# ByeongKyuPark/Depth-Aware-Shader-Effects-for-NeRF

Hardware: AMD Instinct MI355X
Metric: rays/sec at 800x800, 64 coarse + 128 fine samples (higher is better)
Workload: dtype fp32 (f16x3 split)

## Files before the change

depth-aware-shader-effects-for-nerf_amd/csrc/common.h:

```cpp
#pragma once
#include <hip/hip_runtime.h>
#include <stdint.h>
#include <stdio.h>
#include <utility>
#include "../../include/nerfmi_train.h"
#include "layout.h"

namespace nerf {

int set_error(int code, const char* fmt, ...);

inline int check_launch(const char* what) {
  hipError_t e = hipGetLastError();
  if (e != hipSuccess) return set_error(NERF_ERR_HIP, "%s: %s", what, hipGetErrorString(e));
  return NERF_OK;
}

typedef float f32x16 __attribute__((ext_vector_type(16)));
typedef float f32x4 __attribute__((ext_vector_type(4)));

template <typename F, int... Is>
__device__ __forceinline__ void static_for_impl(F&& f, std::integer_sequence<int, Is...>) {
  (f(std::integral_constant<int, Is>{}), ...);
}
template <int N, typename F>
__device__ __forceinline__ void static_for(F&& f) {
  static_for_impl(f, std::make_integer_sequence<int, N>{});
}

__host__ __device__ __forceinline__ int64_t imin64(int64_t a, int64_t b) { return a < b ? a : b; }

__device__ __forceinline__ float opaque_neg_one() {
  float v = -1.0f;
  asm("" : "+s"(v));
  return v;
}
__device__ __forceinline__ _Float16 split_lo(float x, _Float16 hi) {
  return (_Float16)__builtin_fmaf((float)hi, opaque_neg_one(), x);
}

__device__ __forceinline__ uint32_t split_lo_pair(uint32_t hi2, float x0, float x1) {
  uint32_t lo;
  asm("v_fma_mixlo_f16 %0, %1, -1.0, %2 op_sel_hi:[1,0,0]\n\t"
      "v_fma_mixhi_f16 %0, %1, -1.0, %3 op_sel:[1,0,0] op_sel_hi:[1,0,0]"
      : "=&v"(lo)
      : "v"(hi2), "v"(x0), "v"(x1));
  return lo;
}

constexpr int kRowStoreAux = 2;
constexpr int kRowLoadAux = 0;

typedef uint32_t u32x4s __attribute__((ext_vector_type(4)));
template <int AUX, bool PAD = false, typename V>
__device__ __forceinline__ void store16_rows(V v, __amdgpu_buffer_rsrc_t rows, uint32_t voff) {
  static_assert(sizeof(V) == 16, "16-byte stores");
  __builtin_amdgcn_raw_buffer_store_b128(__builtin_bit_cast(u32x4s, v), rows, (int)voff, 0, AUX);
  if constexpr (PAD) asm volatile("s_nop 1");
}

__device__ __forceinline__ float expf_rn(float x) { return (float)exp((double)x); }

__device__ __forceinline__ float wave_max_nn(float v) {
  v = fmaxf(v, __int_as_float(__builtin_amdgcn_mov_dpp(__float_as_int(v), 0xB1, 0xF, 0xF, false)));
  v = fmaxf(v, __int_as_float(__builtin_amdgcn_mov_dpp(__float_as_int(v), 0x4E, 0xF, 0xF, false)));
  v = fmaxf(v, __int_as_float(__builtin_amdgcn_mov_dpp(__float_as_int(v), 0x141, 0xF, 0xF, false)));
  v = fmaxf(v, __int_as_float(__builtin_amdgcn_mov_dpp(__float_as_int(v), 0x140, 0xF, 0xF, false)));
  const float r0 = __int_as_float(__builtin_amdgcn_readlane(__float_as_int(v), 0));
  const float r1 = __int_as_float(__builtin_amdgcn_readlane(__float_as_int(v), 16));
  const float r2 = __int_as_float(__builtin_amdgcn_readlane(__float_as_int(v), 32));
  const float r3 = __int_as_float(__builtin_amdgcn_readlane(__float_as_int(v), 48));
  return fmaxf(fmaxf(r0, r1), fmaxf(r2, r3));
}

__device__ __forceinline__ float block_exp_record(float m) {
  int e;
  frexpf(m, &e);
  return -(float)(kBlockExpBias + (m > 0.0f ? e : kBlockExpZero));
}

__device__ __forceinline__ float hash_uniform(uint64_t seed, uint64_t idx) {
  uint64_t z = seed + 0x9E3779B97F4A7C15ull * (idx + 1);
  z = (z ^ (z >> 30)) * 0xBF58476D1CE4E5B9ull;
  z = (z ^ (z >> 27)) * 0x94D049BB133111EBull;
  z ^= z >> 31;
  return (float)(z >> 40) * (1.0f / 16777216.0f);
}

__host__ __device__ __forceinline__ uint64_t rng_key_at(uint64_t seed, uint64_t first) {
  return seed + 0x9E3779B97F4A7C15ull * first;
}

int launch_get_rays(int H, int W, float focal, const float* c2w, int row0, int nrows,
                    float* o, float* d, hipStream_t s);
int launch_rng_uniforms(uint64_t seed, int64_t first, int64_t n, float* out, hipStream_t s);
int launch_pe(const float* x, int64_t M, int dims, int levels, int include_input, float* out, hipStream_t s);
int launch_normalize(const float* d, int64_t B, float* out, hipStream_t s);
int launch_stratified(const float* o, const float* d, int64_t B, float near_f, float span_f,
                      int N, const float* t_vals, int perturb, const float* t_rand,
                      uint64_t seed, float* z, float* pts, hipStream_t s);
int launch_importance(const float* o, const float* d, const float* z, const float* w,
                      int64_t B, int N, int Nf, const float* u_lin, const float* u_rand,
                      uint64_t seed, float* z_all, float* pts_all, const float* rgb_c, const float* sigma_c,
                      float* rgb_all, float* sigma_all, float* z_fine, int* fine_slot, hipStream_t s,
                      uint16_t* merged_src = nullptr);
int launch_pack(const float* const* params, float* packed, hipStream_t s);
int launch_ray_features(const float* packed, const float* dirs, int64_t R, const float* app,
                        int64_t app_rows, float* feat, hipStream_t s, float* encd = nullptr, float* dn_out = nullptr);
extern int g_mlp_arith;
int launch_mlp16(const float* packed, const float* o, const float* d, const float* z, int64_t R, int N,
                 const float* feat, float* rgb, float* sigma, const int* out_slot, int out_T, hipStream_t s,
                 float* save = nullptr, const float* encd = nullptr, uint32_t* masks = nullptr);
int launch_mlp16_live(const float* packed, const float* o, const float* d, const float* z, int N, const float* feat,
                      const float* encd, const int* live, int64_t M_live, float* rgb, float* sigma, float* rgb_live,
                      float* sigma_live, float* save, uint32_t* masks, hipStream_t s);
int launch_mlp16s(const float* packed, const float* o, const float* d, const float* z, int64_t R, int N,
                  const float* feat, float* rgb, float* sigma, const int* out_slot, int out_T, hipStream_t s);
int launch_mlp16s_live(const float* packed, const float* o, const float* d, const float* z, int64_t R, int N,
                       const float* feat, float* rgb, float* sigma, const int* live, const int* live_count,
                       hipStream_t s);
size_t occ_block_count_bytes(int64_t M);
int launch_occ_classify(const float* o, const float* d, const float* z, int64_t B, int n, const uint32_t* bits, int G,
                        const float* lo, const float* inv, int* live, int* live_count, uint8_t* mask,
                        float* sigma_zero, float* rgb_zero, uint32_t* block_counts, hipStream_t s);
int launch_occ_gather_grads(const float* dsigma, const float* drgb, const int* live, int64_t M_live,
                            float* dsigma_live, float* drgb_live, hipStream_t s);
int launch_occ_pack(const float* lattice, int G, int sp, float thr, uint32_t* bits, hipStream_t s);
int launch_occ_dilate(const uint32_t* in, int G, uint32_t* out, hipStream_t s);
int launch_mlp(const float* packed, const float* o, const float* d, const float* z, int64_t R,
               int N, const float* feat, float* rgb, float* sigma, const int* out_slot, int out_T,
               hipStream_t s, float* save = nullptr, const float* encd = nullptr, uint32_t* masks = nullptr);
struct CompositeSamples {
  const float *rgb, *sigma, *rgb_f, *sigma_f;
  const uint16_t* src;
  const float* z;
  int64_t B;
  int N, Nf;
  bool merged;
};
inline CompositeSamples dense_samples(const float* rgb, const float* sigma, const float* z, int64_t B, int N) {
  return {rgb, sigma, nullptr, nullptr, nullptr, z, B, N, 0, false};
}
inline CompositeSamples merged_samples(const float* rgb_c, const float* sigma_c, const float* rgb_f,
                                       const float* sigma_f, const uint16_t* src, const float* z_all, int64_t B, int N,
                                       int Nf) {
  return {rgb_c, sigma_c, rgb_f, sigma_f, src, z_all, B, N, Nf, true};
}
struct CompositeBg {
  const float* bg;
  int stride;
  float bd;
  float* acc_map;
};
int launch_composite(const CompositeSamples& in, float* rgb_map, float* depth, float* weights, const CompositeBg* bga,
                     hipStream_t s);

}
```

depth-aware-shader-effects-for-nerf_amd/csrc/mlp16s.hip:

```cpp
#include <atomic>
#include "common.h"
#include "pe_sin.h"
#include "stream16.h"

namespace nerf {

#ifdef NERF_MLP16S_STAMPS
__device__ unsigned long long nerf16s_stamps[65536][16];
constexpr int kSStampFloats = kW16Waves * 32;
constexpr int kSStampIter = 8;
#define STAMP16S_ASM(i, insn)                                                               \
  do {                                                                                      \
    __builtin_amdgcn_sched_barrier(0);                                                      \
    unsigned long long t_;                                                                  \
    asm volatile(insn " %0\n\ts_waitcnt lgkmcnt(0)" : "=s"(t_)::"memory");                 \
    __builtin_amdgcn_sched_barrier(0);                                                      \
    if (lane == 0 && stamp_on) reinterpret_cast<unsigned long long*>(lds + kSLdsFloats)[wave * 16 + (i)] = t_; \
  } while (0)
#define STAMP16S(i) STAMP16S_ASM(i, "s_memtime")
#define STAMP16S_REAL(i) STAMP16S_ASM(i, "s_memrealtime")
#else
constexpr int kSStampFloats = 0;
#define STAMP16S(i) do {} while (0)
#define STAMP16S_REAL(i) do {} while (0)
#endif

__device__ __forceinline__ f32x4 mfma16s(h16x8 a, h16x8 b, f32x4 c) {
  return __builtin_amdgcn_mfma_f32_16x16x32_f16(a, b, c, 0, 0, 0);
}

constexpr int kSLdsPe = 4 * kChunkFloats;
constexpr int kSLdsBias = kSLdsPe + kW16Waves * kPeSteps * 64;
constexpr int kSLdsSigmaW = kSLdsBias + 8 * kHidden;
constexpr int kSLdsVecFloats = 8 * kHidden + kHidden + 4;
constexpr int kSLdsConsts = kSLdsBias + kSLdsVecFloats;
constexpr int kSLdsRgb = kSLdsConsts + kS16Consts;
constexpr int kSLdsRgbFloats = 3 * kDirHidden + 4;
constexpr int kSLdsFeat = kSLdsRgb + kSLdsRgbFloats;
constexpr int kSLdsFloats = kSLdsFeat + kW16Waves * kRayFeat;
static_assert(kSLdsRgb % 4 == 0 && kSLdsFeat % 4 == 0, "LDS vector layout");
static_assert((kS16Chunks & (kS16Chunks - 1)) == 0 && kS16Chunks % 4 == 0, "the stream wraps onto the same ring slots");

typedef h16x8 STile[2][2];
typedef f32x4 SAcc[8][2][2];

template <int TI>
__device__ __forceinline__ void sread_tile(const float* slot, const uint32_t (&off)[2], STile& a) {
#pragma unroll
  for (int r = 0; r < 2; ++r)
#pragma unroll
    for (int part = 0; part < 2; ++part)
      a[r][part] = __builtin_bit_cast(h16x8, *reinterpret_cast<const f32x4*>(slot + off[r] + TI * 512 + part * 256));
}

template <int TI, int K>
__device__ __forceinline__ void sread_frag(const float* slot, const uint32_t (&off)[2], STile& a) {
  constexpr int r = K >> 1, part = K & 1;
  a[r][part] = __builtin_bit_cast(h16x8, *reinterpret_cast<const f32x4*>(slot + off[r] + TI * 512 + part * 256));
}

#ifdef NERF16S_PIECE_DMA
constexpr uint32_t kSDmaWave = 1024;
template <int SLOT, int I>
__device__ __forceinline__ void sdma_piece(const float* __restrict__ stream, int c, uint32_t lds_base, uint32_t voff) {
  chunk_dma_piece<SLOT, I>(stream, c, lds_base, voff);
}
#else
constexpr uint32_t kSDmaWave = 4096;
template <int SLOT, int I>
__device__ __forceinline__ void sdma_piece(const float* __restrict__ stream, int c, uint32_t lds_base, uint32_t voff) {
  const char* src = reinterpret_cast<const char*>(stream) + (size_t)c * (kChunkFloats * 4);
  if constexpr (I == 0)
    asm volatile(
        "s_mov_b32 m0, %2\n\t"
        "s_nop 0\n\t"
        "global_load_lds_dwordx4 %0, %1"
        :
        : "v"(voff), "s"(src), "s"(lds_base + SLOT * (kChunkFloats * 4))
        : "memory", "m0");
  else
    asm volatile("global_load_lds_dwordx4 %0, %1 offset:%2" : : "v"(voff), "s"(src), "n"(I * 1024) : "memory");
}
#endif
template <int SLOT>
__device__ __forceinline__ void sdma_chunk(const float* __restrict__ stream, int c, uint32_t lds_base, uint32_t voff) {
  sdma_piece<SLOT, 0>(stream, c, lds_base, voff);
  sdma_piece<SLOT, 1>(stream, c, lds_base, voff);
  sdma_piece<SLOT, 2>(stream, c, lds_base, voff);
  sdma_piece<SLOT, 3>(stream, c, lds_base, voff);
}

template <int G, int TI, bool FIRST, typename Hook>
__device__ __forceinline__ void smfma_tile(const STile& a, const Operand& b0, const Operand& b1, SAcc& acc,
                                           Hook&& hook) {
  static_for<4>([&](auto jc) __attribute__((always_inline)) {
    constexpr int j = decltype(jc)::value, r = j >> 1, st = j & 1;
    const Operand& b = st ? b1 : b0;
    f32x4 c;
    if constexpr (FIRST) c = mfma16s(a[r][1], b.hi, f32x4{});
    else c = mfma16s(a[r][1], b.hi, acc[4 * G + TI][r][st]);
    c = mfma16s(a[r][0], b.lo, c);
    acc[4 * G + TI][r][st] = mfma16s(a[r][0], b.hi, c);
    hook(jc);
  });
}

constexpr int kSValuGap0 = 5;
template <int G, int TI, bool FIRST, int NRD, int VPG, typename Reads, typename Side, typename Hook>
__device__ __forceinline__ void ssegment(const STile& a, const Operand& b0, const Operand& b1, SAcc& acc, Reads&& reads,
                                         Side&& side, Hook&& hook) {
  side(std::integral_constant<int, 0>{});
  __builtin_amdgcn_sched_barrier(0);
  reads();
  smfma_tile<G, TI, FIRST>(a, b0, b1, acc, hook);
  side(std::integral_constant<int, 1>{});
#pragma unroll
  for (int i = 0; i < 12; ++i) {
    __builtin_amdgcn_sched_group_barrier(0x008, 1, 0);
    if (i >= 1 && i <= 4 * NRD) __builtin_amdgcn_sched_group_barrier(0x100, 1, 0);
    if (VPG > 0 && i >= kSValuGap0) __builtin_amdgcn_sched_group_barrier(0x002, VPG, 0);
  }
  __builtin_amdgcn_sched_barrier(0);
}

__device__ __forceinline__ constexpr int shalf_unit_at(int gap, int slot, bool two) {
  if (two) return gap >= 5 + slot && gap <= 10 + slot ? gap - 5 - slot : -2;
  return slot ? -2 : (gap >= 5 && gap <= 7 ? gap - 5 : (gap >= 9 && gap <= 11 ? gap - 6 : -2));
}
template <int G, int TI, bool FIRST, int NRD, bool TWO, typename Frag, typename Side, typename Hook>
__device__ __forceinline__ void ssegment_h(const STile& a, const Operand& b0, const Operand& b1, SAcc& acc, Frag&& frag,
                                           Side&& side, Hook&& hook) {
  using Slot0 = std::integral_constant<int, 0>;
  using Slot1 = std::integral_constant<int, 1>;
  side(Slot0{}, std::integral_constant<int, -1>{});
  side(Slot1{}, std::integral_constant<int, -1>{});
  __builtin_amdgcn_sched_barrier(0);
  static_for<12>([&](auto ic) __attribute__((always_inline)) {
    constexpr int i = decltype(ic)::value, j = i / 3, k = i % 3, r = j >> 1, st = j & 1;
    const Operand& b = st ? b1 : b0;
    f32x4& c = acc[4 * G + TI][r][st];
    if constexpr (k == 0) c = FIRST ? mfma16s(a[r][1], b.hi, f32x4{}) : mfma16s(a[r][1], b.hi, c);
    if constexpr (k == 1) c = mfma16s(a[r][0], b.lo, c);
    if constexpr (k == 2) {
      c = mfma16s(a[r][0], b.hi, c);
      hook(std::integral_constant<int, j>{});
    }
    if constexpr (i >= 1 && i <= 4 * NRD) frag(std::integral_constant<int, i - 1>{});
    side(Slot0{}, std::integral_constant<int, shalf_unit_at(i, 0, TWO)>{});
    side(Slot1{}, std::integral_constant<int, shalf_unit_at(i, 1, TWO)>{});
    __builtin_amdgcn_sched_barrier(0);
  });
}

enum SSide { kSNone, kSPrev, kSCur, kSL0, kSSkipPrev, kSSkipCur, kSPrevPe, kSCurPe, kSPrevH, kSCurH };
__device__ __forceinline__ constexpr int spe_at(int i, int seg) {
  return (i == 7 || i == 8) && (seg == 0 || seg == 2) ? 2 * (i - 7) + seg / 2 : -1;
}
__device__ __forceinline__ constexpr int sq_prev(int i, int seg) {
  constexpr int base[7] = {0, 3, 6, 8, 10, 12, 14};
  if (i >= 7) return -1;
  const int n = i < 2 ? 3 : 2;
  if (n == 3) return seg >= 1 ? base[i] + seg - 1 : -1;
  return seg == 1 ? base[i] : (seg == 3 ? base[i] + 1 : -1);
}
__device__ __forceinline__ constexpr int sq_cur(int i, int seg) {
  constexpr int base[8] = {0, 0, 2, 4, 6, 8, 11, 14};
  constexpr int cnt[8] = {0, 2, 2, 2, 2, 3, 3, 2};
  if (i >= 8 || cnt[i] == 0) return -1;
  if (cnt[i] == 3) return seg >= 1 ? base[i] + seg - 1 : -1;
  return seg == 1 ? base[i] : (seg == 3 ? base[i] + 1 : -1);
}
__device__ __forceinline__ constexpr int sh_prev(int i, int seg, int slot) {
  if (i == 0) return 2 * seg + slot;
  return i >= 7 || slot ? -1 : 8 + 4 * (i - 1) + seg;
}
__device__ __forceinline__ constexpr int sh_cur(int i, int seg, int slot) {
  if (i == 7) return 24 + 2 * seg + slot;
  return i == 0 || i >= 8 || slot ? -1 : 4 * (i - 1) + seg;
}
__device__ __forceinline__ constexpr bool sh_schedules_hold() {
  int np = 0, nc = 0;
  for (int i = 0; i < 8; ++i)
    for (int seg = 0; seg < 4; ++seg)
      for (int slot = 0; slot < 2; ++slot) {
        const int hp = sh_prev(i, seg, slot), hc = sh_cur(i, seg, slot);
        if (hp >= 0 && (hp != np++ || i >= 4 + hp / 8)) return false;
        if (hc >= 0 && (hc != nc++ || i <= hc / 8)) return false;
      }
  return np == 32 && nc == 32;
}
static_assert(sh_schedules_hold(), "half-quarter schedules: each half once, in order, inside its window");
template <bool CUR>
__device__ __forceinline__ constexpr int spe_next(int i, int seg) {
  if (i >= 8 || (CUR ? sq_cur(i, seg) : sq_prev(i, seg)) >= 0) return -1;
  int n = 0;
  for (int k = 0; k < 4 * i + seg; ++k) n += (CUR ? sq_cur(k / 4, k % 4) : sq_prev(k / 4, k % 4)) < 0;
  return n + (CUR ? 0 : 16);
}
static_assert(spe_next<true>(7, 2) == 15 && spe_next<false>(7, 3) == 31, "32 free segments");
template <int KIND>
__device__ __forceinline__ constexpr int side_count(int i, int seg) {
  if constexpr (KIND == kSPrevPe || KIND == kSCurPe) return 1;
  if constexpr (KIND == kSPrev) return sq_prev(i, seg) >= 0;
  if constexpr (KIND == kSSkipPrev) return (sq_prev(i, seg) >= 0) + (spe_at(i, seg) >= 0);
  if constexpr (KIND == kSCur) return sq_cur(i, seg) >= 0;
  if constexpr (KIND == kSSkipCur) return (sq_cur(i, seg) >= 0) + (spe_at(i, seg) >= 0);
  if constexpr (KIND == kSL0) return 2;
  return 0;
}
template <int KIND>
__device__ __forceinline__ constexpr int svpg(int i, int seg) {
  const int n = side_count<KIND>(i, seg);
  return n == 0 ? 0 : (n * 40 + 11 - kSValuGap0) / (12 - kSValuGap0);
}

template <int G, int TI, bool FIRST, int NRD, int KIND, int I, typename Frag, typename Side, typename Hook>
__device__ __forceinline__ void sseg(const STile& a, const Operand& b0, const Operand& b1, SAcc& acc, Frag&& frag,
                                     Side&& side, Hook&& hook) {
  using IC = std::integral_constant<int, I>;
  using SC = std::integral_constant<int, TI>;
  if constexpr (KIND == kSPrevH || KIND == kSCurH) {
    constexpr bool two = (KIND == kSPrevH ? sh_prev(I, TI, 1) : sh_cur(I, TI, 1)) >= 0;
    ssegment_h<G, TI, FIRST, NRD, two>(a, b0, b1, acc, frag, [&](auto slot, auto unit) __attribute__((always_inline)) {
      side(IC{}, SC{}, slot, unit);
    }, hook);
  } else {
    ssegment<G, TI, FIRST, NRD, svpg<KIND>(I, TI)>(a, b0, b1, acc, [&]() __attribute__((always_inline)) {
      static_for<4>(frag);
    }, [&](auto ph) __attribute__((always_inline)) { side(IC{}, SC{}, ph); }, hook);
  }
}

struct SNoPub {
  template <typename I>
  __device__ __forceinline__ void operator()(I) const {}
};
template <int G, int SLOT, bool FIRST, int TAIL, int KIND, int I, bool WRAP, typename Side, typename Pub>
__device__ __forceinline__ void schunk(const float* __restrict__ stream, int c, float* lds, uint32_t lds_dma,
                                       uint32_t voff, const uint32_t (&off)[2], STile (&a)[4], const Operand& b0,
                                       const Operand& b1, SAcc& acc, Side&& side, Pub&& pub) {
  const float* cur = lds + SLOT * kChunkFloats;
  const float* nxt = lds + ((SLOT + 1) & 3) * kChunkFloats;
  auto none = [](auto) {};
  using S0 = std::integral_constant<int, 0>;
  using S1 = std::integral_constant<int, 1>;
  using S2 = std::integral_constant<int, 2>;
  using S3 = std::integral_constant<int, 3>;
  sseg<G, 0, FIRST, 1, KIND, I>(a[0], b0, b1, acc, [&](auto kc) __attribute__((always_inline)) {
    sread_frag<3, decltype(kc)::value>(cur, off, a[3]);
  }, side, none);
  if constexpr (TAIL >= 1) {
    wait_vmcnt<TAIL >= 2 ? 4 : 0>();
    __builtin_amdgcn_s_barrier();
  }
  pub(std::integral_constant<int, I>{});
  auto dma = [&](auto pc) __attribute__((always_inline)) {
    if constexpr (TAIL >= 3)
      sdma_piece<(SLOT + 3) & 3, decltype(pc)::value>(stream, WRAP ? (c + 3) & (kS16Chunks - 1) : c + 3, lds_dma, voff);
  };
  sseg<G, 1, FIRST, (TAIL >= 1), KIND, I>(a[1], b0, b1, acc, [&](auto kc) __attribute__((always_inline)) {
    if constexpr (TAIL >= 1) sread_frag<0, decltype(kc)::value>(nxt, off, a[0]);
  }, side, [&](auto jc) __attribute__((always_inline)) {
    if constexpr (decltype(jc)::value == 0) dma(S0{});
    if constexpr (decltype(jc)::value == 2) dma(S1{});
  });
  sseg<G, 2, FIRST, (TAIL >= 1), KIND, I>(a[2], b0, b1, acc, [&](auto kc) __attribute__((always_inline)) {
    if constexpr (TAIL >= 1) sread_frag<1, decltype(kc)::value>(nxt, off, a[1]);
  }, side, [&](auto jc) __attribute__((always_inline)) {
    if constexpr (decltype(jc)::value == 0) dma(S2{});
  });
  sseg<G, 3, FIRST, (TAIL >= 1), KIND, I>(a[3], b0, b1, acc, [&](auto kc) __attribute__((always_inline)) {
    if constexpr (TAIL >= 1) sread_frag<2, decltype(kc)::value>(nxt, off, a[2]);
  }, side, [&](auto jc) __attribute__((always_inline)) {
    if constexpr (decltype(jc)::value == 0) dma(S3{});
  });
}

template <int G, int NSTEP, int SLOT0, int TAIL_END, int KIND, bool WRAP = false, typename Opnd, typename Side,
          typename Pub = SNoPub>
__device__ __forceinline__ void sgroup(const float* __restrict__ stream, int c0, float* lds, uint32_t lds_dma,
                                       uint32_t voff, const uint32_t (&off)[2], STile (&a)[4], SAcc& acc,
                                       Opnd&& operand, Side&& side, Pub&& pub = Pub{}) {
  static_for<NSTEP>([&](auto ic) __attribute__((always_inline)) {
    constexpr int i = decltype(ic)::value;
    constexpr int left = NSTEP - 1 - i + TAIL_END;
    schunk<G, (SLOT0 + i) & 3, i == 0, (left < 3 ? left : 3), KIND, i, WRAP>(
        stream, c0 + i, lds, lds_dma, voff, off, a, operand(ic, std::integral_constant<int, 0>{}),
        operand(ic, std::integral_constant<int, 1>{}), acc, side, pub);
  });
}

__device__ __forceinline__ float smax4(float m) {
  m = fmaxf(m, __shfl_xor(m, 16));
  return fmaxf(m, __shfl_xor(m, 32));
}
__device__ __forceinline__ float ssum4(float v) {
  v = v + __shfl_xor(v, 16);
  return v + __shfl_xor(v, 32);
}

struct SQuarter {
  f32x4 b, w;
};

template <int PH, int T0, int QG, bool SIGMA>
__device__ __forceinline__ void squarter(const SAcc& acc, const float (&inv)[2], const float* bias, const float* ws,
                                         int nlane, const float (&sc)[2], Operand (&in)[16], float (&m)[2],
                                         float (&part)[2], SQuarter& qv) {
  constexpr int T = T0 + QG / 4, r = (QG % 4) >> 1, st = QG & 1;
  const int n0 = 32 * T + 8 * r + nlane;
  if constexpr (PH == 0) {
    qv.b = *reinterpret_cast<const f32x4*>(bias + n0);
    if constexpr (SIGMA) qv.w = *reinterpret_cast<const f32x4*>(ws + n0);
  } else {
    float xs[4];
#pragma unroll
    for (int e = 0; e < 4; ++e) {
      const float y = fmaxf(fmaf(acc[T][r][st][e], inv[st], qv.b[e]), 0.0f);
      m[st] = fmaxf(m[st], y);
      if constexpr (SIGMA) part[st] = fmaf(qv.w[e], y, part[st]);
      xs[e] = y * sc[st];
    }
    Operand& op = in[2 * T + st];
    typedef _Float16 h16x2 __attribute__((ext_vector_type(2)));
#pragma unroll
    for (int p = 0; p < 2; ++p) {
      const h16x2 hi2 = {(_Float16)xs[2 * p], (_Float16)xs[2 * p + 1]};
      const h16x2 lo2 = __builtin_bit_cast(h16x2, split_lo_pair(__builtin_bit_cast(uint32_t, hi2), xs[2 * p], xs[2 * p + 1]));
      const int j = 4 * r + 2 * p;
      op.hi[j] = hi2[0];
      op.hi[j + 1] = hi2[1];
      op.lo[j] = lo2[0];
      op.lo[j + 1] = lo2[1];
    }
  }
}

__device__ __forceinline__ void sunpaired(float& v, float after) {
#ifndef NERF16S_PACKED_SIDE
  asm("" : "+v"(v) : "v"(after));
#endif
}

typedef float f32x2s __attribute__((ext_vector_type(2)));
struct SHalf {
  f32x2s b;
  float y[2], xs[2];
};

template <int U, int T0, int H>
__device__ __forceinline__ void shalf(const SAcc& acc, const float (&inv)[2], const float* bias, int nlane,
                                      const float (&sc)[2], Operand (&in)[16], float (&m)[2], SHalf& hv) {
  constexpr int QG = H >> 1, p = H & 1, T = T0 + QG / 4, r = (QG % 4) >> 1, st = QG & 1, j = 4 * r + 2 * p;
  typedef _Float16 h16x2 __attribute__((ext_vector_type(2)));
  Operand& op = in[2 * T + st];
  if constexpr (U == -1) hv.b = *reinterpret_cast<const f32x2s*>(bias + 32 * T + 8 * r + nlane + 2 * p);
  if constexpr (U == 0) {
    hv.y[0] = fmaf(acc[T][r][st][2 * p], inv[st], hv.b[0]);
    float b1 = hv.b[1];
    sunpaired(b1, hv.y[0]);
    hv.b[1] = b1;
  }
  if constexpr (U == 1) {
    hv.y[1] = fmaf(acc[T][r][st][2 * p + 1], inv[st], hv.b[1]);
    hv.y[0] = fmaxf(hv.y[0], 0.0f);
  }
  if constexpr (U == 2) {
    hv.y[1] = fmaxf(hv.y[1], 0.0f);
    hv.xs[0] = hv.y[0] * sc[st];
    sunpaired(hv.y[1], hv.xs[0]);
  }
  if constexpr (U == 3) {
    hv.xs[1] = hv.y[1] * sc[st];
    m[st] = fmaxf(fmaxf(m[st], hv.y[0]), hv.y[1]);
  }
  if constexpr (U == 4) {
    const h16x2 hi2 = {(_Float16)hv.xs[0], (_Float16)hv.xs[1]};
    op.hi[j] = hi2[0];
    op.hi[j + 1] = hi2[1];
  }
  if constexpr (U == 5) {
    const h16x2 hi2 = {op.hi[j], op.hi[j + 1]};
    const h16x2 lo2 = __builtin_bit_cast(h16x2, split_lo_pair(__builtin_bit_cast(uint32_t, hi2), hv.xs[0], hv.xs[1]));
    op.lo[j] = lo2[0];
    op.lo[j + 1] = lo2[1];
  }
}

template <int U>
__device__ __forceinline__ void shalf_follow(const SHalf& first, SHalf& second) {
  if constexpr (U == 1) sunpaired(second.y[0], first.xs[0]);
  if constexpr (U == 2) sunpaired(second.y[1], first.xs[1]);
}

template <int PH, int t, int st>
__device__ __forceinline__ void spe_operand(const float* pe_mine, const float (&sc)[2], Operand& op, float (&v)[8],
                                            int lane) {
  if constexpr (PH == 0) {
#pragma unroll
    for (int j = 0; j < 8; ++j) v[j] = pe_mine[((st * 2 + t) * 8 + j) * 64 + lane];
  } else {
#pragma unroll
    for (int j = 0; j < 8; ++j) split_into(v[j] * sc[st], op, j);
  }
}

#define MLP16S_GATHER 0
#include "mlp16s_body.h"
#undef MLP16S_GATHER
#define MLP16S_GATHER 1
#include "mlp16s_body.h"
#undef MLP16S_GATHER

static int device_cus() {
  static std::atomic<int> cached[64];
  int dev = 0;
  if (hipGetDevice(&dev) != hipSuccess || dev < 0 || dev >= 64) return 0;
  int n = cached[dev].load(std::memory_order_relaxed);
  if (n == 0) {
    if (hipDeviceGetAttribute(&n, hipDeviceAttributeMultiprocessorCount, dev) != hipSuccess || n <= 0) return 0;
    cached[dev].store(n, std::memory_order_relaxed);
  }
  return n;
}

int launch_mlp16s(const float* packed, const float* o, const float* d, const float* z, int64_t R, int N,
                  const float* feat, float* rgb, float* sigma, const int* out_slot, int out_T, hipStream_t s) {
  const int64_t M = R * (int64_t)N;
  if (M == 0) return NERF_OK;
  constexpr int per_block = 32 * kW16Waves;
  const int64_t blocks = (M + per_block - 1) / per_block;
  const int cus = device_cus();
  if (cus <= 0) return set_error(NERF_ERR_HIP, "mlp16s_kernel: cannot read the device's CU count");
  hipLaunchKernelGGL(mlp16s_kernel, dim3((unsigned)(blocks < cus ? blocks : cus)), dim3(64 * kW16Waves), 0, s, packed, o, d, z, M, N, feat,
                     rgb, sigma, out_slot, out_T);
  return check_launch("mlp16s_kernel");
}

int launch_mlp16s_live(const float* packed, const float* o, const float* d, const float* z, int64_t R, int N,
                       const float* feat, float* rgb, float* sigma, const int* live, const int* live_count,
                       hipStream_t s) {
  const int64_t M = R * (int64_t)N;
  if (M == 0) return NERF_OK;
  constexpr int per_block = 32 * kW16Waves;
  const int64_t blocks = (M + per_block - 1) / per_block;
  const int cus = device_cus();
  if (cus <= 0) return set_error(NERF_ERR_HIP, "mlp16s_live_kernel: cannot read the device's CU count");
  hipLaunchKernelGGL(mlp16s_live_kernel, dim3((unsigned)(blocks < cus ? blocks : cus)), dim3(64 * kW16Waves), 0, s,
                     packed, o, d, z, N, feat, rgb, sigma, live, live_count);
  return check_launch("mlp16s_live_kernel");
}

}
```

depth-aware-shader-effects-for-nerf_amd/csrc/mlp16s_body.h:

```cpp
__global__ void __launch_bounds__(64 * kW16Waves, 1)
#if MLP16S_GATHER
mlp16s_live_kernel(const float* __restrict__ packed, const float* __restrict__ orig, const float* __restrict__ dirs,
                   const float* __restrict__ zv, int N, const float* __restrict__ feat, float* __restrict__ rgb,
                   float* __restrict__ sigma, const int* __restrict__ live, const int* __restrict__ live_count) {
#else
mlp16s_kernel(const float* __restrict__ packed, const float* __restrict__ orig, const float* __restrict__ dirs,
              const float* __restrict__ zv, int64_t M, int N, const float* __restrict__ feat,
              float* __restrict__ rgb, float* __restrict__ sigma, const int* __restrict__ out_slot, int out_T) {
#endif
  __shared__ __attribute__((aligned(16))) float lds[kSLdsFloats + kSStampFloats];
  const int wave = __builtin_amdgcn_readfirstlane(threadIdx.x >> 6), lane0 = threadIdx.x & 63;
#if MLP16S_GATHER
  const int64_t M = *live_count;
  if ((int64_t)blockIdx.x * (32 * kW16Waves) >= M) return;
  const int* const out_slot = nullptr;
  constexpr int out_T = 0;
#endif
  const int mlast = (int)(M - 1);
  const int nblk = (int)((M + 32 * kW16Waves - 1) / (32 * kW16Waves));
  int blk = blockIdx.x;
  auto sample_of = [&](int b, int st) {
    return imin64(((int64_t)b * kW16Waves + wave) * 32 + 16 * st + (lane0 & 15), (int64_t)mlast);
  };
  float in_z[2], in_o[2][3], in_d[2][3];
#if MLP16S_GATHER
  int sm_cur[2], sm_n[2];
  auto load_live = [&](int b, int (&sm)[2]) __attribute__((always_inline)) {
#pragma unroll
    for (int st = 0; st < 2; ++st) sm[st] = live[sample_of(b, st)];
  };
  auto load_inputs = [&](const int (&sml)[2]) __attribute__((always_inline)) {
#pragma unroll
    for (int st = 0; st < 2; ++st) {
      const int sm = sml[st];
#else
  auto load_inputs = [&](int b) __attribute__((always_inline)) {
#pragma unroll
    for (int st = 0; st < 2; ++st) {
      const int sm = (int)sample_of(b, st);
#endif
      const int64_t row = zv ? sm / N : sm;
#pragma unroll
      for (int c = 0; c < 3; ++c) in_o[st][c] = orig[3 * row + c];
      in_z[st] = 0.0f;
#pragma unroll
      for (int c = 0; c < 3; ++c) in_d[st][c] = 0.0f;
      if (zv) {
        in_z[st] = zv[sm];
#pragma unroll
        for (int c = 0; c < 3; ++c) in_d[st][c] = dirs[3 * row + c];
      }
    }
  };
  float x[2][3];
  auto positions = [&](float (&x)[2][3]) __attribute__((always_inline)) {
#pragma unroll
    for (int st = 0; st < 2; ++st)
#pragma unroll
      for (int c = 0; c < 3; ++c) {
        const float p = in_o[st][c] + in_d[st][c] * in_z[st];
        x[st][c] = zv ? p : in_o[st][c];
      }
  };
#if MLP16S_GATHER
  load_live(blk, sm_cur);
  load_inputs(sm_cur);
#else
  load_inputs(blk);
#endif
  positions(x);
  for (int i = threadIdx.x; i < kSLdsVecFloats / 4; i += 64 * kW16Waves)
    reinterpret_cast<f32x4*>(lds + kSLdsBias)[i] = reinterpret_cast<const f32x4*>(packed + kOffBias)[i];
  if (threadIdx.x < kS16Consts) lds[kSLdsConsts + threadIdx.x] = packed[kOffScale16 + threadIdx.x];
  if (threadIdx.x < kSLdsRgbFloats / 4)
    reinterpret_cast<f32x4*>(lds + kSLdsRgb)[threadIdx.x] = reinterpret_cast<const f32x4*>(packed + kOffRgbW)[threadIdx.x];
  __builtin_amdgcn_s_waitcnt(0);
  __builtin_amdgcn_sched_barrier(0);
  const float* stream = packed + kOff16;
  uint32_t lds_dma = (uint32_t)(uintptr_t)(lptr_t)lds + kSDmaWave * wave;
  auto fragment_offsets = [](int l, uint32_t (&off)[2]) __attribute__((always_inline)) {
    const int li = l & 15, hh = (l >> 4) & 1, ss = l >> 5;
#pragma unroll
    for (int r = 0; r < 2; ++r) off[r] = (uint32_t)(ss * 2048 + 4 * ((li & 7) + 8 * r + 16 * (li >> 3) + 32 * hh));
  };
  float* pe_mine = lds + kSLdsPe + wave * kPeSteps * 64;
  const float* bias = lds + kSLdsBias;
  const float* ws = lds + kSLdsSigmaW;
  const float* cst = lds + kSLdsConsts;
#if MLP16S_GATHER
  constexpr bool one_ray = false;
#else
  const bool one_ray = (N & 31) == 0;
#endif
  float* feat_mine = lds + kSLdsFeat + wave * kRayFeat;
  STile a[4];
  {
    const uint32_t voff = 16u * lane0 + kSDmaWave * wave;
    sdma_chunk<0>(stream, 0, lds_dma, voff);
    sdma_chunk<1>(stream, 1, lds_dma, voff);
    sdma_chunk<2>(stream, 2, lds_dma, voff);
    uint32_t off[2];
    fragment_offsets(lane0, off);
    wait_vmcnt<8>();
    __builtin_amdgcn_s_barrier();
    sread_tile<0>(lds, off, a[0]);
    sread_tile<1>(lds, off, a[1]);
    sread_tile<2>(lds, off, a[2]);
  }

  Operand pe_op[4];
  bool full = true;
#ifdef NERF_MLP16S_STAMPS
  int it = 0;
#endif
#pragma unroll 1
  for (;;) {
  asm volatile("" : "+s"(stream));
  asm volatile("" : "+s"(lds_dma));
  int lane = lane0;
  asm volatile("" : "+v"(lane));
  const int g = lane >> 4, li = lane & 15, hh = g & 1, ss = g >> 1;
  const uint32_t voff = 16u * lane + kSDmaWave * wave;
  uint32_t off[2];
  fragment_offsets(lane, off);
  const int nlane = 4 * hh + 16 * ss;
#ifdef NERF_MLP16S_STAMPS
  const bool stamp_on = it == kSStampIter || (it < kSStampIter && blk + (int)gridDim.x >= nblk);
  ++it;
#endif
  STAMP16S(0);
  STAMP16S_REAL(12);
  const int64_t s0 = ((int64_t)blk * kW16Waves + wave) * 32;

  auto pe_arg = [&](const float (&xa)[2][3], int st, int p) __attribute__((always_inline)) {
    const int fi = p / 3, fc = p - 3 * fi;
    const float xc = fc == 0 ? xa[st][0] : (fc == 1 ? xa[st][1] : xa[st][2]);
    return xc * __int_as_float((127 + (fi < kPosLevels ? fi : 0)) << 23);
  };
  auto pe_tail = [&](const float (&xa)[2][3], int st, int p, float v) __attribute__((always_inline)) {
    return p < 3 * kPosLevels ? v : (p == 30 ? (hh ? xa[st][1] : xa[st][0]) : (hh ? 0.0f : xa[st][2]));
  };
  auto pe_beyond = [&](const float (&xa)[2][3]) __attribute__((always_inline)) {
    float ax = 0.0f;
#pragma unroll
    for (int st = 0; st < 2; ++st)
      ax = fmaxf(ax, fmaxf(fabsf(xa[st][0]), fmaxf(fabsf(xa[st][1]), fabsf(xa[st][2]))));
    return __any(ax * (float)(1 << (kPosLevels - 1)) > kPeSinMax) != 0;
  };
  auto pe_bound = [&](const float (&xa)[2][3], int st) __attribute__((always_inline)) {
    return fmaxf(1.0f, fmaxf(fabsf(xa[st][0]), fmaxf(fabsf(xa[st][1]), fabsf(xa[st][2]))));
  };
  float m_pe[2];
  float s_cur[2], inv_cur[2], s_nxt[2], inv_prev[2], m[2] = {0.0f, 0.0f}, part[2] = {0.0f, 0.0f};
#pragma unroll
  for (int st = 0; st < 2; ++st) {
    m_pe[st] = pe_bound(x, st);
    s_cur[st] = pow2_scale(m_pe[st]);
  }
  if (full) {
    float pe[2][2][8];
    if (pe_beyond(x)) {
#pragma unroll
      for (int st = 0; st < 2; ++st)
#pragma unroll
        for (int t = 0; t < 2; ++t)
#pragma unroll
          for (int j = 0; j < 8; ++j) {
            const int p = 8 * (2 * t + ss) + j;
            float sn, cs;
            sincosf(pe_arg(x, st, p), &sn, &cs);
            pe[st][t][j] = pe_tail(x, st, p, hh ? cs : sn);
          }
    } else {
#pragma unroll
      for (int st = 0; st < 2; ++st)
#pragma unroll
        for (int t = 0; t < 2; ++t)
#pragma unroll
          for (int j = 0; j < 8; ++j) {
            const int p = 8 * (2 * t + ss) + j;
            pe[st][t][j] = pe_tail(x, st, p, pe_sin_reduced(pe_arg(x, st, p), hh));
          }
    }
#pragma unroll
    for (int st = 0; st < 2; ++st)
#pragma unroll
      for (int t = 0; t < 2; ++t)
#pragma unroll
        for (int j = 0; j < 8; ++j) {
          pe_mine[((st * 2 + t) * 8 + j) * 64 + lane] = pe[st][t][j];
          split_into(pe[st][t][j] * s_cur[st], pe_op[2 * t + st], j);
        }
  }
  const int nxt_blk = blk + (int)gridDim.x;
  float xn[2][3], s_n[2];
  bool beyond_n = false;
  Operand pe_nx[4];
  int lane_n = lane;
  auto pub_next = [&](auto ic) __attribute__((always_inline)) {
#if MLP16S_GATHER
    if constexpr (decltype(ic)::value == 0) load_live(nxt_blk, sm_n);
    if constexpr (decltype(ic)::value == 1) load_inputs(sm_n);
    if constexpr (decltype(ic)::value == 3) {
#else
    if constexpr (decltype(ic)::value == 0) load_inputs(nxt_blk);
    if constexpr (decltype(ic)::value == 2) {
#endif
      asm volatile("" : "+v"(lane_n));
      positions(xn);
#pragma unroll
      for (int st = 0; st < 2; ++st) s_n[st] = pow2_scale(pe_bound(xn, st));
      beyond_n = pe_beyond(xn);
    }
  };
  auto side_pe_next = [&](auto nc, auto ph) __attribute__((always_inline)) {
    constexpr int n = decltype(nc)::value;
    if constexpr (n >= 0 && decltype(ph)::value == 1) {
      constexpr int st = n >> 4, t = (n >> 3) & 1, j = n & 7;
      constexpr int p0 = 16 * t + j, p1 = p0 + 8;
      constexpr int f0 = p0 / 3, c0 = p0 % 3, f1 = p1 / 3 < kPosLevels ? p1 / 3 : 0, c1 = p1 % 3;
      const bool upper = lane_n >= 32;
      const int hn = (lane_n >> 4) & 1;
      const float a0 = xn[st][c0] * (float)(1 << f0), a1 = xn[st][c1] * (float)(1 << f1);
      const float r = pe_sin_reduced(upper ? a1 : a0, hn);
      float v = r;
      if constexpr (p1 == 30) v = upper ? (hn ? xn[st][1] : xn[st][0]) : r;
      if constexpr (p1 == 31) v = upper ? (hn ? 0.0f : xn[st][2]) : r;
      pe_mine[((st * 2 + t) * 8 + j) * 64 + lane_n] = v;
      split_into(v * s_n[st], pe_nx[2 * t + st], j);
      asm volatile("" : "+v"(pe_nx[2 * t + st].hi), "+v"(pe_nx[2 * t + st].lo));
    }
  };
  SAcc acc;
  Operand in[16];
#pragma unroll
  for (int st = 0; st < 2; ++st) {
    inv_cur[st] = cst[kS16InvW + 0] / s_cur[st];
    s_nxt[st] = pow2_scale(cst[kS16R + 0] * m_pe[st] + cst[kS16B + 0]);
  }
  SQuarter qv[2];
  SHalf hv[2];
  float pe_v[8];
  auto pe_operand_of = [&](auto i, auto st) -> const Operand& {
    return pe_op[2 * decltype(i)::value + decltype(st)::value];
  };

  STAMP16S(1);
  sgroup<0, 2, 0, 3, kSNone>(stream, 0, lds, lds_dma, voff, off, a, acc, pe_operand_of,
                             [](auto, auto, auto) {});
  sgroup<1, 2, 2, 3, kSL0>(stream, 2, lds, lds_dma, voff, off, a, acc, pe_operand_of,
                           [&](auto i, auto seg, auto ph) __attribute__((always_inline)) {
                             constexpr int q0 = 8 * decltype(i)::value + 2 * decltype(seg)::value;
                             squarter<decltype(ph)::value, 0, q0, false>(acc, inv_cur, bias, ws, nlane, s_nxt, in, m,
                                                                         part, qv[0]);
                             squarter<decltype(ph)::value, 0, q0 + 1, false>(acc, inv_cur, bias, ws, nlane, s_nxt, in,
                                                                             m, part, qv[1]);
                           });

  STAMP16S(2);
#pragma unroll
  for (int st = 0; st < 2; ++st) {
    inv_prev[st] = inv_cur[st];
    s_cur[st] = s_nxt[st];
  }
  const float* bias_prev = bias;
  auto act_operand = [&](auto i, auto st) -> const Operand& { return in[2 * decltype(i)::value + decltype(st)::value]; };
  auto op4 = [&](auto i, auto st) -> const Operand& {
    constexpr int k = decltype(i)::value, t = decltype(st)::value;
    if constexpr (k < 8) return in[2 * k + t];
    else return pe_op[2 * (k - 8) + t];
  };
  auto side_prev = [&](auto i, auto seg, auto ph, auto sigma_tag) __attribute__((always_inline)) {
    constexpr int q = sq_prev(decltype(i)::value, decltype(seg)::value);
    if constexpr (q >= 0)
      squarter<decltype(ph)::value, 4, q, decltype(sigma_tag)::value>(acc, inv_prev, bias_prev, ws, nlane, s_cur, in, m,
                                                                       part, qv[0]);
  };
  auto side_cur = [&](auto i, auto seg, auto ph, const float* bias_l, auto sigma_tag) __attribute__((always_inline)) {
    constexpr int q = sq_cur(decltype(i)::value, decltype(seg)::value);
    if constexpr (q >= 0)
      squarter<decltype(ph)::value, 0, q, decltype(sigma_tag)::value>(acc, inv_cur, bias_l, ws, nlane, s_nxt, in, m,
                                                                      part, qv[1]);
  };
  auto side_prev_h = [&](auto i, auto seg, auto slot, auto unit) __attribute__((always_inline)) {
    constexpr int h = sh_prev(decltype(i)::value, decltype(seg)::value, decltype(slot)::value);
    if constexpr (h >= 0 && decltype(unit)::value >= -1)
      shalf<decltype(unit)::value, 4, h>(acc, inv_prev, bias_prev, nlane, s_cur, in, m, hv[decltype(slot)::value]);
    if constexpr (decltype(slot)::value == 1 && h >= 0)
      shalf_follow<decltype(unit)::value>(hv[0], hv[1]);
  };
  auto side_cur_h = [&](auto i, auto seg, auto slot, auto unit, const float* bias_l) __attribute__((always_inline)) {
    constexpr int h = sh_cur(decltype(i)::value, decltype(seg)::value, decltype(slot)::value);
    if constexpr (h >= 0 && decltype(unit)::value >= -1)
      shalf<decltype(unit)::value, 0, h>(acc, inv_cur, bias_l, nlane, s_nxt, in, m, hv[decltype(slot)::value]);
    if constexpr (decltype(slot)::value == 1 && h >= 0)
      shalf_follow<decltype(unit)::value>(hv[0], hv[1]);
  };
#ifdef NERF16S_QUARTER_SIDE
  constexpr int kKindPrev = kSPrev, kKindCur = kSCur;
#else
  constexpr int kKindPrev = kSPrevH, kKindCur = kSCurH;
#endif
  float s_pe[2] = {0.0f, 0.0f};
  auto side_pe = [&](auto i, auto seg, auto ph) __attribute__((always_inline)) {
    constexpr int k = spe_at(decltype(i)::value, decltype(seg)::value);
    if constexpr (k >= 0) spe_operand<decltype(ph)::value, k / 2, k % 2>(pe_mine, s_pe, pe_op[k], pe_v, lane);
  };
  using NoSigma = std::false_type;
  using Sigma = std::true_type;
  auto layer = [&](int L, auto skip_tag, auto sg_tag, auto&& pub_a) __attribute__((always_inline)) {
    constexpr bool SKIP = decltype(skip_tag)::value;
    constexpr bool SG = decltype(sg_tag)::value;
#pragma unroll
    for (int st = 0; st < 2; ++st) {
      inv_cur[st] = cst[kS16InvW + L] / s_cur[st];
      if constexpr (SKIP) s_pe[st] = s_cur[st];
    }
    const float* bias_l = bias + L * kHidden;
    const int c0 = s16_chunk0(1) + (L - 1) * 16 + (L > kSkipLayer ? 4 : 0);
    if constexpr (SKIP) {
      sgroup<0, 10, 0, 3, kSSkipPrev>(stream, c0, lds, lds_dma, voff, off, a, acc, op4,
                                      [&](auto i, auto seg, auto ph) __attribute__((always_inline)) {
                                        side_prev(i, seg, ph, NoSigma{});
                                        side_pe(i, seg, ph);
                                      });
    } else {
      sgroup<0, 8, 0, 3, kKindPrev>(stream, c0, lds, lds_dma, voff, off, a, acc, act_operand,
                                    [&](auto i, auto seg, auto... at) __attribute__((always_inline)) {
                                      if constexpr (sizeof...(at) == 2) side_prev_h(i, seg, at...);
                                      else side_prev(i, seg, at..., NoSigma{});
                                    }, pub_a);
    }
#pragma unroll
    for (int st = 0; st < 2; ++st) {
      const float ms = smax4(m[st]);
      float bound = cst[kS16R + L] * (SKIP ? fmaxf(ms, m_pe[st]) : ms) + cst[kS16B + L];
      if (L + 1 == kSkipLayer) bound = fmaxf(bound, m_pe[st]);
      s_nxt[st] = pow2_scale(bound);
      m[st] = 0.0f;
    }
    if constexpr (SKIP) {
      sgroup<1, 10, 2, 3, kSSkipCur>(stream, c0 + 10, lds, lds_dma, voff, off, a, acc, op4,
                                     [&](auto i, auto seg, auto ph) __attribute__((always_inline)) {
                                       side_cur(i, seg, ph, bias_l, NoSigma{});
                                       side_pe(i, seg, ph);
                                     });
    } else {
      sgroup<1, 8, 0, 3, SG ? kSCurPe : kKindCur>(
          stream, c0 + 8, lds, lds_dma, voff, off, a, acc, act_operand,
          [&](auto i, auto seg, auto... at) __attribute__((always_inline)) {
            if constexpr (sizeof...(at) == 2) {
              side_cur_h(i, seg, at..., bias_l);
            } else {
              side_cur(i, seg, at..., bias_l, sg_tag);
              if constexpr (SG)
                side_pe_next(std::integral_constant<int, spe_next<true>(decltype(i)::value, decltype(seg)::value)>{},
                             at...);
            }
          });
    }
#pragma unroll
    for (int st = 0; st < 2; ++st) {
      inv_prev[st] = inv_cur[st];
      s_cur[st] = s_nxt[st];
    }
    bias_prev = bias_l;
    STAMP16S(2 + L);
  };
#pragma unroll 1
  for (int L = 1; L < kSkipLayer; ++L) layer(L, NoSigma{}, NoSigma{}, SNoPub{});
  layer(kSkipLayer, Sigma{}, NoSigma{}, SNoPub{});
#pragma unroll 1
  for (int L = kSkipLayer + 1; L < 7; ++L) layer(L, NoSigma{}, NoSigma{}, SNoPub{});
  layer(7, NoSigma{}, Sigma{}, pub_next);

  if (one_ray) {
    const char* src = reinterpret_cast<const char*>(feat + (imin64(s0, M - 1) / N) * kRayFeat);
    const uint32_t dst = (uint32_t)(uintptr_t)(lptr_t)feat_mine;
    uint32_t keep;
    asm volatile(
        "s_mov_b32 %0, m0\n\t"
        "s_mov_b32 m0, %3\n\t"
        "s_nop 0\n\t"
        "global_load_lds_dwordx4 %1, %2\n\t"
        "s_mov_b32 m0, %0"
        : "=&s"(keep)
        : "v"(16u * lane), "s"(src), "s"(dst)
        : "memory");
  }
#pragma unroll
  for (int st = 0; st < 2; ++st) inv_cur[st] = cst[kS16InvW + 8] / s_cur[st];
  sgroup<0, 8, 0, 3, kSPrevPe, true>(
      stream, s16_chunk0(8), lds, lds_dma, voff, off, a, acc, act_operand,
      [&](auto i, auto seg, auto ph) __attribute__((always_inline)) {
        side_prev(i, seg, ph, Sigma{});
        side_pe_next(std::integral_constant<int, spe_next<false>(decltype(i)::value, decltype(seg)::value)>{}, ph);
      });

  STAMP16S(10);
  float sig[2];
#pragma unroll
  for (int st = 0; st < 2; ++st) sig[st] = fmaxf(ssum4(part[st]) + ws[kHidden], 0.0f);
  const float* wr = lds + kSLdsRgb;
  float pr[2][3] = {{0.0f, 0.0f, 0.0f}, {0.0f, 0.0f, 0.0f}};
  auto colour_head = [&](const float* fr, int st) __attribute__((always_inline)) {
#pragma unroll
    for (int T = 0; T < 4; ++T)
#pragma unroll
      for (int r = 0; r < 2; ++r) {
        const int n0 = 32 * T + 8 * r + nlane;
        const f32x4 fd = *reinterpret_cast<const f32x4*>(fr + n0);
        const f32x4 ap = *reinterpret_cast<const f32x4*>(fr + kDirHidden + n0);
        f32x4 hd;
#pragma unroll
        for (int e = 0; e < 4; ++e) hd[e] = fmaxf(fmaf(acc[T][r][st][e], inv_cur[st], fd[e]), 0.0f) + ap[e];
#pragma unroll
        for (int c = 0; c < 3; ++c) {
          const f32x4 w = *reinterpret_cast<const f32x4*>(wr + c * kDirHidden + n0);
#pragma unroll
          for (int e = 0; e < 4; ++e) pr[st][c] = fmaf(w[e], hd[e], pr[st][c]);
        }
      }
  };
  if (one_ray) wait_vmcnt<8>();
  if (one_ray) {
    colour_head(feat_mine, 0);
    colour_head(feat_mine, 1);
  } else {
#if MLP16S_GATHER
    colour_head(feat + (int64_t)(sm_cur[0] / N) * kRayFeat, 0);
    colour_head(feat + (int64_t)(sm_cur[1] / N) * kRayFeat, 1);
#else
    colour_head(feat + (int64_t)((int)sample_of(blk, 0) / N) * kRayFeat, 0);
    colour_head(feat + (int64_t)((int)sample_of(blk, 1) / N) * kRayFeat, 1);
#endif
  }
  float out[3];
#pragma unroll
  for (int c = 0; c < 3; ++c) {
    const float v0 = ssum4(pr[0][c]) + wr[3 * kDirHidden + c], v1 = ssum4(pr[1][c]) + wr[3 * kDirHidden + c];
    const float v = (g & 1) ? v1 : v0;
    out[c] = 1.0f / (1.0f + expf_rn(-v));
  }
  if (g < 2) {
    const int st = g;
    if (s0 + 16 * st + li < M) {
#if MLP16S_GATHER
      const int sm = st ? sm_cur[1] : sm_cur[0];
#else
      const int sm = (int)(s0 + 16 * st + li);
#endif
      const int64_t o_s = out_slot ? (int64_t)(sm / N) * out_T + out_slot[sm] : (int64_t)sm;
      sigma[o_s] = st ? sig[1] : sig[0];
#pragma unroll
      for (int c = 0; c < 3; ++c) rgb[3 * o_s + c] = out[c];
    }
  }
  STAMP16S(11);
  STAMP16S_REAL(13);
  if (nxt_blk >= nblk) break;
  blk = nxt_blk;
  full = beyond_n;
#pragma unroll
  for (int k = 0; k < 4; ++k) pe_op[k] = pe_nx[k];
#pragma unroll
  for (int st = 0; st < 2; ++st)
#pragma unroll
    for (int c = 0; c < 3; ++c) x[st][c] = xn[st][c];
#if MLP16S_GATHER
  sm_cur[0] = sm_n[0];
  sm_cur[1] = sm_n[1];
#endif
  }
  wait_vmcnt<0>();
#ifdef NERF_MLP16S_STAMPS
  if (const int64_t w_ = (int64_t)blockIdx.x * kW16Waves + wave; w_ < 65536 && lane0 == 0)
    for (int i = 0; i < 16; ++i)
      nerf16s_stamps[w_][i] = reinterpret_cast<const unsigned long long*>(lds + kSLdsFloats)[wave * 16 + i];
#endif
}
```

Baseline: 2.284 million.

## Cut index and scale arithmetic in the fp16-split MLP kernel

```diff
diff --git a/depth-aware-shader-effects-for-nerf_amd/csrc/common.h b/depth-aware-shader-effects-for-nerf_amd/csrc/common.h
--- a/depth-aware-shader-effects-for-nerf_amd/csrc/common.h
+++ b/depth-aware-shader-effects-for-nerf_amd/csrc/common.h
@@ -5,6 +5,7 @@
 #include <utility>
 #include "../../include/nerfmi_train.h"
 #include "layout.h"
+#include "sample_index.h"
 
 namespace nerf {
 
diff --git a/depth-aware-shader-effects-for-nerf_amd/csrc/mlp16s.hip b/depth-aware-shader-effects-for-nerf_amd/csrc/mlp16s.hip
--- a/depth-aware-shader-effects-for-nerf_amd/csrc/mlp16s.hip
+++ b/depth-aware-shader-effects-for-nerf_amd/csrc/mlp16s.hip
@@ -290,13 +290,35 @@
   });
 }
 
+__device__ __forceinline__ void sacc_hold(SAcc& acc) {
+#ifndef NERF16S_EDGE_BURST
+#pragma unroll
+  for (int T = 4; T < 8; ++T)
+#pragma unroll
+    for (int r = 0; r < 2; ++r)
+#pragma unroll
+      for (int st = 0; st < 2; ++st) asm volatile("" : "+a"(acc[T][r][st]));
+#endif
+}
+
+typedef unsigned u32x2s __attribute__((ext_vector_type(2)));
+template <typename F>
+__device__ __forceinline__ float sover4(float v, F&& f) {
+#ifdef NERF16S_SHFL_REDUCE
+  v = f(v, __shfl_xor(v, 16));
+  return f(v, __shfl_xor(v, 32));
+#else
+  const u32x2s a = __builtin_amdgcn_permlane16_swap(__float_as_uint(v), __float_as_uint(v), false, false);
+  v = f(__uint_as_float(a[0]), __uint_as_float(a[1]));
+  const u32x2s b = __builtin_amdgcn_permlane32_swap(__float_as_uint(v), __float_as_uint(v), false, false);
+  return f(__uint_as_float(b[0]), __uint_as_float(b[1]));
+#endif
+}
 __device__ __forceinline__ float smax4(float m) {
-  m = fmaxf(m, __shfl_xor(m, 16));
-  return fmaxf(m, __shfl_xor(m, 32));
+  return sover4(m, [](float x, float y) { return fmaxf(x, y); });
 }
 __device__ __forceinline__ float ssum4(float v) {
-  v = v + __shfl_xor(v, 16);
-  return v + __shfl_xor(v, 32);
+  return sover4(v, [](float x, float y) { return x + y; });
 }
 
 struct SQuarter {
@@ -432,8 +454,9 @@
   const int64_t blocks = (M + per_block - 1) / per_block;
   const int cus = device_cus();
   if (cus <= 0) return set_error(NERF_ERR_HIP, "mlp16s_kernel: cannot read the device's CU count");
+  const RayDiv nd = ray_div_of(N);
   hipLaunchKernelGGL(mlp16s_kernel, dim3((unsigned)(blocks < cus ? blocks : cus)), dim3(64 * kW16Waves), 0, s, packed, o, d, z, M, N, feat,
-                     rgb, sigma, out_slot, out_T);
+                     rgb, sigma, out_slot, out_T, nd.mul, nd.shift);
   return check_launch("mlp16s_kernel");
 }
 
@@ -446,8 +469,9 @@
   const int64_t blocks = (M + per_block - 1) / per_block;
   const int cus = device_cus();
   if (cus <= 0) return set_error(NERF_ERR_HIP, "mlp16s_live_kernel: cannot read the device's CU count");
+  const RayDiv nd = ray_div_of(N);
   hipLaunchKernelGGL(mlp16s_live_kernel, dim3((unsigned)(blocks < cus ? blocks : cus)), dim3(64 * kW16Waves), 0, s,
-                     packed, o, d, z, N, feat, rgb, sigma, live, live_count);
+                     packed, o, d, z, N, feat, rgb, sigma, live, live_count, nd.mul, nd.shift);
   return check_launch("mlp16s_live_kernel");
 }
 
diff --git a/depth-aware-shader-effects-for-nerf_amd/csrc/mlp16s_body.h b/depth-aware-shader-effects-for-nerf_amd/csrc/mlp16s_body.h
--- a/depth-aware-shader-effects-for-nerf_amd/csrc/mlp16s_body.h
+++ b/depth-aware-shader-effects-for-nerf_amd/csrc/mlp16s_body.h
@@ -2,11 +2,13 @@
 #if MLP16S_GATHER
 mlp16s_live_kernel(const float* __restrict__ packed, const float* __restrict__ orig, const float* __restrict__ dirs,
                    const float* __restrict__ zv, int N, const float* __restrict__ feat, float* __restrict__ rgb,
-                   float* __restrict__ sigma, const int* __restrict__ live, const int* __restrict__ live_count) {
+                   float* __restrict__ sigma, const int* __restrict__ live, const int* __restrict__ live_count,
+                   uint32_t n_mul, int n_shift) {
 #else
 mlp16s_kernel(const float* __restrict__ packed, const float* __restrict__ orig, const float* __restrict__ dirs,
               const float* __restrict__ zv, int64_t M, int N, const float* __restrict__ feat,
-              float* __restrict__ rgb, float* __restrict__ sigma, const int* __restrict__ out_slot, int out_T) {
+              float* __restrict__ rgb, float* __restrict__ sigma, const int* __restrict__ out_slot, int out_T,
+              uint32_t n_mul, int n_shift) {
 #endif
   __shared__ __attribute__((aligned(16))) float lds[kSLdsFloats + kSStampFloats];
   const int wave = __builtin_amdgcn_readfirstlane(threadIdx.x >> 6), lane0 = threadIdx.x & 63;
@@ -20,9 +22,27 @@
   const int nblk = (int)((M + 32 * kW16Waves - 1) / (32 * kW16Waves));
   int blk = blockIdx.x;
   auto sample_of = [&](int b, int st) {
-    return imin64(((int64_t)b * kW16Waves + wave) * 32 + 16 * st + (lane0 & 15), (int64_t)mlast);
+    const uint32_t i = ((uint32_t)b * kW16Waves + wave) * 32 + 16 * st + (lane0 & 15);
+    return (int)(i < (uint32_t)mlast ? i : (uint32_t)mlast);
+  };
+  auto ray_of = [&](int sm) {
+#ifdef NERF16S_DIV_INDEX
+    return sm / N;
+#else
+    return ray_div(sm, n_mul, n_shift);
+#endif
+  };
+  auto over_scale = [](float c, float s) {
+#ifdef NERF16S_IEEE_INV
+    return c / s;
+#else
+    return c * pow2_recip(s);
+#endif
   };
   float in_z[2], in_o[2][3], in_d[2][3];
+  const int pt_mask = zv ? 0 : -1;
+  const float* const z_or = zv ? zv : orig;
+  const float* const d_or = zv ? dirs : orig;
 #if MLP16S_GATHER
   int sm_cur[2], sm_n[2];
   auto load_live = [&](int b, int (&sm)[2]) __attribute__((always_inline)) {
@@ -37,19 +57,14 @@
   auto load_inputs = [&](int b) __attribute__((always_inline)) {
 #pragma unroll
     for (int st = 0; st < 2; ++st) {
-      const int sm = (int)sample_of(b, st);
-#endif
-      const int64_t row = zv ? sm / N : sm;
+      const int sm = sample_of(b, st);
+#endif
+      const int64_t row = (ray_of(sm) & ~pt_mask) | (sm & pt_mask);
 #pragma unroll
       for (int c = 0; c < 3; ++c) in_o[st][c] = orig[3 * row + c];
-      in_z[st] = 0.0f;
-#pragma unroll
-      for (int c = 0; c < 3; ++c) in_d[st][c] = 0.0f;
-      if (zv) {
-        in_z[st] = zv[sm];
-#pragma unroll
-        for (int c = 0; c < 3; ++c) in_d[st][c] = dirs[3 * row + c];
-      }
+      in_z[st] = z_or[sm];
+#pragma unroll
+      for (int c = 0; c < 3; ++c) in_d[st][c] = d_or[3 * row + c];
     }
   };
   float x[2][3];
@@ -59,7 +74,7 @@
 #pragma unroll
       for (int c = 0; c < 3; ++c) {
         const float p = in_o[st][c] + in_d[st][c] * in_z[st];
-        x[st][c] = zv ? p : in_o[st][c];
+        x[st][c] = pt_mask ? in_o[st][c] : p;
       }
   };
 #if MLP16S_GATHER
@@ -130,7 +145,7 @@
 #endif
   STAMP16S(0);
   STAMP16S_REAL(12);
-  const int64_t s0 = ((int64_t)blk * kW16Waves + wave) * 32;
+  const uint32_t s0 = ((uint32_t)blk * kW16Waves + wave) * 32;
 
   auto pe_arg = [&](const float (&xa)[2][3], int st, int p) __attribute__((always_inline)) {
     const int fi = p / 3, fc = p - 3 * fi;
@@ -207,6 +222,10 @@
     if constexpr (decltype(ic)::value == 2) {
 #endif
       asm volatile("" : "+v"(lane_n));
+#pragma unroll
+      for (int st = 0; st < 2; ++st)
+        asm volatile("" : "+v"(in_z[st]), "+v"(in_o[st][0]), "+v"(in_o[st][1]), "+v"(in_o[st][2]), "+v"(in_d[st][0]),
+                     "+v"(in_d[st][1]), "+v"(in_d[st][2]));
       positions(xn);
 #pragma unroll
       for (int st = 0; st < 2; ++st) s_n[st] = pow2_scale(pe_bound(xn, st));
@@ -235,7 +254,7 @@
   Operand in[16];
 #pragma unroll
   for (int st = 0; st < 2; ++st) {
-    inv_cur[st] = cst[kS16InvW + 0] / s_cur[st];
+    inv_cur[st] = over_scale(cst[kS16InvW + 0], s_cur[st]);
     s_nxt[st] = pow2_scale(cst[kS16R + 0] * m_pe[st] + cst[kS16B + 0]);
   }
   SQuarter qv[2];
@@ -311,9 +330,10 @@
   auto layer = [&](int L, auto skip_tag, auto sg_tag, auto&& pub_a) __attribute__((always_inline)) {
     constexpr bool SKIP = decltype(skip_tag)::value;
     constexpr bool SG = decltype(sg_tag)::value;
+    sacc_hold(acc);
 #pragma unroll
     for (int st = 0; st < 2; ++st) {
-      inv_cur[st] = cst[kS16InvW + L] / s_cur[st];
+      inv_cur[st] = over_scale(cst[kS16InvW + L], s_cur[st]);
       if constexpr (SKIP) s_pe[st] = s_cur[st];
     }
     const float* bias_l = bias + L * kHidden;
@@ -374,8 +394,15 @@
   for (int L = kSkipLayer + 1; L < 7; ++L) layer(L, NoSigma{}, NoSigma{}, SNoPub{});
   layer(7, NoSigma{}, Sigma{}, pub_next);
 
+#if MLP16S_GATHER
   if (one_ray) {
-    const char* src = reinterpret_cast<const char*>(feat + (imin64(s0, M - 1) / N) * kRayFeat);
+#elif defined(NERF16S_DMA_BRANCH)
+  if (one_ray) {
+#else
+  {
+#endif
+    const int first = (int)(s0 < (uint32_t)mlast ? s0 : (uint32_t)mlast);
+    const char* src = reinterpret_cast<const char*>(feat + (int64_t)ray_of(first) * kRayFeat);
     const uint32_t dst = (uint32_t)(uintptr_t)(lptr_t)feat_mine;
     uint32_t keep;
     asm volatile(
@@ -388,8 +415,9 @@
         : "v"(16u * lane), "s"(src), "s"(dst)
         : "memory");
   }
-#pragma unroll
-  for (int st = 0; st < 2; ++st) inv_cur[st] = cst[kS16InvW + 8] / s_cur[st];
+  sacc_hold(acc);
+#pragma unroll
+  for (int st = 0; st < 2; ++st) inv_cur[st] = over_scale(cst[kS16InvW + 8], s_cur[st]);
   sgroup<0, 8, 0, 3, kSPrevPe, true>(
       stream, s16_chunk0(8), lds, lds_dma, voff, off, a, acc, act_operand,
       [&](auto i, auto seg, auto ph) __attribute__((always_inline)) {
@@ -428,11 +456,11 @@
     colour_head(feat_mine, 1);
   } else {
 #if MLP16S_GATHER
-    colour_head(feat + (int64_t)(sm_cur[0] / N) * kRayFeat, 0);
-    colour_head(feat + (int64_t)(sm_cur[1] / N) * kRayFeat, 1);
-#else
-    colour_head(feat + (int64_t)((int)sample_of(blk, 0) / N) * kRayFeat, 0);
-    colour_head(feat + (int64_t)((int)sample_of(blk, 1) / N) * kRayFeat, 1);
+    colour_head(feat + (int64_t)ray_of(sm_cur[0]) * kRayFeat, 0);
+    colour_head(feat + (int64_t)ray_of(sm_cur[1]) * kRayFeat, 1);
+#else
+    colour_head(feat + (int64_t)ray_of(sample_of(blk, 0)) * kRayFeat, 0);
+    colour_head(feat + (int64_t)ray_of(sample_of(blk, 1)) * kRayFeat, 1);
 #endif
   }
   float out[3];
@@ -444,13 +472,13 @@
   }
   if (g < 2) {
     const int st = g;
-    if (s0 + 16 * st + li < M) {
+    if (s0 + 16 * st + li <= (uint32_t)mlast) {
 #if MLP16S_GATHER
       const int sm = st ? sm_cur[1] : sm_cur[0];
 #else
       const int sm = (int)(s0 + 16 * st + li);
 #endif
-      const int64_t o_s = out_slot ? (int64_t)(sm / N) * out_T + out_slot[sm] : (int64_t)sm;
+      const int64_t o_s = out_slot ? (int64_t)ray_of(sm) * out_T + out_slot[sm] : (int64_t)sm;
       sigma[o_s] = st ? sig[1] : sig[0];
 #pragma unroll
       for (int c = 0; c < 3; ++c) rgb[3 * o_s + c] = out[c];
diff --git a/depth-aware-shader-effects-for-nerf_amd/csrc/sample_index.h b/depth-aware-shader-effects-for-nerf_amd/csrc/sample_index.h
--- /dev/null
+++ b/depth-aware-shader-effects-for-nerf_amd/csrc/sample_index.h
@@ -0,0 +1,25 @@
+#pragma once
+#include <stdint.h>
+#include "layout.h"
+
+namespace nerf {
+
+struct RayDiv {
+  uint32_t mul;
+  int shift;
+};
+inline RayDiv ray_div_of(int d) {
+  int l = 0;
+  while (((int64_t)1 << l) < d) ++l;
+  const uint64_t p = (uint64_t)1 << (31 + l);
+  return {(uint32_t)((p + (uint64_t)d - 1) / (uint64_t)d), l};
+}
+NERF_HD inline int ray_div(int n, uint32_t mul, int shift) {
+  return (int)((uint32_t)(((uint64_t)((uint32_t)n << 1) * mul) >> 32) >> shift);
+}
+
+NERF_HD inline float pow2_recip(float s) {
+  return __builtin_bit_cast(float, 0x7F000000u - __builtin_bit_cast(uint32_t, s));
+}
+
+}
```

Result: faster. 2.321 million (median of 6 runs) (+1.6%).
